# archinetai/audio-diffusion-pytorch

Hardware: AMD Instinct MI355X
Metric: denoising steps/s (UNetV0 fwd+bwd) at [B,2,2**18] (higher is better)
Workload: dtype f32; 1 GPU; BASELINE.json configs[1]: unconditional DiffusionModel(UNetV0 channels=[8,32,64,128,256,512,512,1024,1024], factors=[1,4,4,4,2,2,2,2,2], items=[1,2,2,2,2,2,2,4,4]) fwd+bwd, audio=randn(4,2,2**18) per GPU, random-init weights; per_gpu_batch=4, global_batch=4, length=262144, launch=hipGraph replay, parallelism=single, collective_world_size=1, collectives_in_graph=False, optimizer=none (the metric is fwd+bwd; gradients for all 176M parameters are produced)

## Files before the change

audio_diffusion_pytorch_amd/_C.py:

```python
import ctypes
import os
from ctypes import POINTER, Structure, c_float, c_int, c_int64, c_void_p

import torch

_PKG_DIR = os.path.dirname(os.path.abspath(__file__))
LIB_PATH = os.path.join(_PKG_DIR, "libadp_hip.so")

_lib = None
_allow_cpu = False

ERRORS = {-1: "bad shape", -2: "unsupported configuration", -3: "misaligned pointer", -4: "kernel launch failed",
          -5: "null pointer"}

P = c_void_p
I = c_int64
F = c_float


class ConvDesc(Structure):
    _fields_ = [(n, c_void_p) for n in ("x", "x2", "w", "bias", "pro_stats", "pro_gamma", "pro_beta", "e_scale",
                                        "res", "out", "out_pre")] + \
               [(n, c_int64) for n in ("B", "R", "R1", "Lin", "M", "N", "KT", "stride", "dil", "pad", "up",
                                       "transposed", "prologue", "groups", "store", "sp", "e_bstride")] + \
# ... 79 lines not shown
    "adp_tflat_out_len": (I, [I, I, I]),
    "adp_tflat_fwd": (c_int, [P, P, I, I, I, I, I, P, P]),
    "adp_tflat_wgrad_ws_bytes": (I, [I, I, I, I, I]),
    "adp_tflat_wgrad": (c_int, [P, P, I, I, I, I, I, P, P, P]),
    "adp_ctx_fold_fwd": (c_int, [P, P, P, I, I, I, P, P, P]),
    "adp_ctx_fold_bwd": (c_int, [P, P, P, P, P, I, I, I, P, P, P, P]),
    "adp_attn_fwd": (c_int, [P, P, P, I, I, I, I, I, I, I, P, P, P, P]),
    "adp_attn_fwd_ws_bytes": (I, [I, I, I, I, I]),
    "adp_attn_bwd_ws_bytes": (I, [I, I, I, I, I]),
    "adp_attn_bwd": (c_int, [P, P, P, P, P, P, I, I, I, I, I, I, I, P, P, P, P, P]),
    "adp_probe_copy": (c_int, [P, P, I, P]),
    "adp_probe_mfma": (I, [I, P, I, P]),
    "adp_probe_launch": (c_int, [I, P]),
    "adp_probe_chase": (c_int, [P, I, P, P]),
    "adp_probe_copy_v": (c_int, [P, P, I, c_int, P]),
    "adp_probe_mfma_v": (I, [I, P, I, c_int, P]),
}

ABI["adp_ar.h"] = {
    "adp_arv_noise": (c_int, [P, P, P, I, I, I, I, P, P, P, P]),
    "adp_arv_step": (c_int, [P, P, P, I, I, I, I, P, P, P]),
    "adp_arv_plane": (c_int, [P, I, I, I, P, P]),
}

ABI["adp_lt.h"] = {
    "adp_lt_conv_out_len": (I, [I, I, I, I]),
    "adp_lt_convt_out_len": (I, [I, I, I, I]),
    "adp_lt_conv": (c_int, [P, P, I, I, I, I, I, I, I, I, P, P]),
    "adp_lt_convt": (c_int, [P, P, I, I, I, I, I, I, I, I, I, P, P]),
    "adp_lt_wgrad_ws_bytes": (I, [I, I, I, I, I]),
    "adp_lt_wgrad": (c_int, [P, P, I, I, I, I, I, I, I, I, I, P, P, P]),
}

ABI["adp_enc.h"] = {
    "adp_enc_down_out_len": (I, [I, I]),
    "adp_enc_down_fwd": (c_int, [P, P, P, I, I, I, I, I, P, P]),
    "adp_enc_down_dgrad": (c_int, [P, P, I, I, I, I, I, P, P]),
    "adp_enc_down_wgrad_ws_bytes": (I, [I, I, I, I, I]),
    "adp_enc_down_wgrad": (c_int, [P, P, I, I, I, I, I, P, P, P, P]),
    "adp_enc_tanh_fwd": (c_int, [P, I, P, P]),
    "adp_enc_tanh_bwd": (c_int, [P, P, I, P, P]),
}

ABI["adp_t5.h"] = {
    "adp_t5_embed": (c_int, [P, P, I, I, I, P, P]),
    "adp_t5_rmsnorm": (c_int, [P, P, I, I, F, P, P]),
    "adp_t5_linear_ws_bytes": (I, [I, I, I]),
    "adp_t5_linear": (c_int, [P, P, P, I, I, I, I, P, P, P]),
    "adp_t5_attn": (c_int, [P, P, P, P, I, I, I, I, I, P, P]),
}

ABI["adp_rng.h"] = {
    "adp_philox_bits": (c_int, [P, I, P, P]),
    "adp_randn": (c_int, [P, I, P, P]),
    "adp_v_inpaint_step_rng": (c_int, [P, P, P, P, P, P, I, P, P]),
}

ABI["adp_clip.h"] = {
    "adp_clip_ws_bytes": (I, [I, I]),
    "adp_clip_scale": (c_int, [P, P, P, I, I, I, F, F, P, P, P]),
    "adp_clip_apply": (c_int, [P, P, I, I, P, P]),
    "adp_clip_step": (c_int, [P, P, P, P, P, I, P, I, I, P, P, P, P]),
}

ABI["adp_gated.h"] = {
    "adp_gated_linear_ws_bytes": (I, [I, I, I]),
    "adp_gated_linear": (c_int, [P, P, P, I, I, I, I, P, P, P]),
}

ABI["adp_sde.h"] = {
    "adp_v_step_eta": (c_int, [P, P, P, P, I, P, I, I, P, P]),
}

ABI["adp_rf.h"] = {
    "adp_rf_noise": (c_int, [P, P, P, I, I, P, P, P]),
    "adp_rf_step": (c_int, [P, P, P, P, I, I, P, I, I, P, P, P]),
}

ABI["adp_edm.h"] = {
    "adp_edm_noise": (c_int, [P, P, P, F, I, I, P, P, P]),
    "adp_edm_step": (c_int, [P, P, P, P, P, I, I, P, I, I, P, P, P]),
}


HEADER_SOURCE = {"adp_ar.h": "elementwise.hip", "adp_lt.h": "lt.hip", "adp_enc.h": "encoder.hip", "adp_t5.h": "t5.hip",
                 "adp_rng.h": "rng.hip", "adp_clip.h": "clip.hip", "adp_gated.h": "gated.hip", "adp_sde.h": "sde.hip",
                 "adp_rf.h": "rf.hip", "adp_edm.h": "edm.hip"}

SIGNATURES = {}
for _header, _table in ABI.items():
    for _name in _table:
        if _name in SIGNATURES:
            _first = next(h for h, t in ABI.items() if _name in t)
            raise ImportError(f"{_name} is in the tables of both {_first} and {_header}: one header declares an entry point")
    SIGNATURES.update(_table)


def _bind(path: str):
    lib = ctypes.CDLL(path)
    for name, (res, args) in SIGNATURES.items():
        fn = getattr(lib, name)
        fn.restype = res
        fn.argtypes = args
    return lib


def lib():
    global _lib
    if _lib is None:
        if not os.path.exists(LIB_PATH):
            raise RuntimeError(
                f"{LIB_PATH} is missing: build the gfx950 kernels first "
                "(python -m audio_diffusion_pytorch_amd.build or __graft_entry__.build()); "
                "audio_diffusion_pytorch_amd has no CPU/PyTorch fallback path")
        _lib = _bind(LIB_PATH)
    return _lib


def _testing_use_library(path, allow_cpu: bool):
    global _lib, _allow_cpu
    _lib = _bind(path) if path is not None else None
    _allow_cpu = allow_cpu


def stream() -> int:
    if _allow_cpu and not torch.cuda.is_available():
        return 0
    return torch.cuda.current_stream().cuda_stream


def ptr(t, dtype=torch.float32):
    if t is None:
        return None
    if t.dtype != dtype:
        raise TypeError(f"adp kernel argument must be {dtype}; got {t.dtype}")
    if not t.is_contiguous():
        raise ValueError("adp kernels need contiguous tensors")
    if not t.is_cuda and not _allow_cpu:
        raise RuntimeError("adp kernels run on MI355X (HIP) tensors only; got a CPU tensor and there is no CPU path")
    return t.data_ptr()


def check(code: int, what: str):
    if code != 0:
        raise RuntimeError(f"{what} failed: {ERRORS.get(code, code)} ({code})")


PROFILE = None
_TAG = None
REPLAY = None


def tag(**meta):
    global _TAG
    if PROFILE is not None:
        _TAG = meta


def _decode_trace(text: str) -> str:
    import re
    names = []
    for item in text.split("\n"):
        if not item:
            continue
        kern, _, site = item.partition("@")
        kern = kern.strip()
        while kern.startswith("(") and kern.endswith(")"):
            kern = kern[1:-1].strip()
        m = re.search(r"\[(?:with )?([^\]]*)\]\s*$", site)
        env = {}
# ... 60 lines not shown
```

audio_diffusion_pytorch_amd/build.py:

```python
import glob
import os
import subprocess
import sys

PKG_DIR = os.path.dirname(os.path.abspath(__file__))
REPO_ROOT = os.path.dirname(PKG_DIR)
CSRC = os.path.join(PKG_DIR, "csrc")
LIB_PATH = os.path.join(PKG_DIR, "libadp_hip.so")
SOURCES = ["conv1d.hip", "conv_mm.hip", "conv_mm_m64.hip", "conv_mm_m32.hip", "conv_tile.hip", "conv_tilek.hip", "conv_tilek1.hip", "conv_mm4.hip", "wgrad_mm.hip", "conv_direct.hip", "wgrad_direct.hip", "norm.hip", "elementwise.hip", "resample.hip", "linear.hip", "attention.hip", "ctx_bank.hip", "lt.hip", "encoder.hip", "t5.hip", "gated.hip", "rng.hip", "clip.hip", "sde.hip", "rf.hip", "edm.hip", "probe.hip"]


def _newest_mtime(paths):
    return max(os.path.getmtime(p) for p in paths)


def sources():
    return [os.path.join(CSRC, s) for s in SOURCES if os.path.exists(os.path.join(CSRC, s))]


def headers():
    return sorted(glob.glob(os.path.join(CSRC, "*.h")) + glob.glob(os.path.join(REPO_ROOT, "include", "*.h")))


def build(force: bool = False, verbose: bool = True) -> str:
    srcs = sources()
    deps = srcs + headers()
    if not force and os.path.exists(LIB_PATH) and os.path.getmtime(LIB_PATH) >= _newest_mtime(deps):
        return LIB_PATH
    hipcc = os.environ.get("HIPCC", "/opt/rocm/bin/hipcc")
    objs = []
    procs = []
    os.makedirs(os.path.join(PKG_DIR, "build"), exist_ok=True)
    for s in srcs:
        o = os.path.join(PKG_DIR, "build", os.path.basename(s) + ".o")
        objs.append(o)
        if not force and os.path.exists(o) and os.path.getmtime(o) >= _newest_mtime([s] + deps[len(srcs):]):
            continue
        cmd = [hipcc, "--offload-arch=gfx950", "-O3", "-std=c++17", "-fPIC", "-c", "-x", "hip", s, "-o", o,
               "-I", os.path.join(REPO_ROOT, "include"), "-I", CSRC, "-Wno-unused-value"]
        if verbose:
            print("[adp build]", " ".join(cmd), flush=True)
        procs.append((cmd, subprocess.Popen(cmd)))
    for cmd, p in procs:
        if p.wait() != 0:
            raise RuntimeError("hipcc failed: " + " ".join(cmd))
    cmd = [hipcc, "--offload-arch=gfx950", "-shared", "-fPIC", "-o", LIB_PATH] + objs
    if verbose:
        print("[adp build]", " ".join(cmd), flush=True)
    subprocess.check_call(cmd)
    return LIB_PATH


if __name__ == "__main__":
    build(force="--force" in sys.argv)
```

audio_diffusion_pytorch_amd/ops.py:

```python
import contextlib
import ctypes
import os
from ctypes import byref
from typing import Optional, Tuple

import torch
from torch import Tensor

from . import _C
from ._C import ConvDesc, WgradDesc, ptr

GN_EPS = 1e-5
MODULATION_LN_EPS = 1e-5
ATTENTION_LN_EPS = 1e-5


def _ws(nbytes: int, like: Tensor) -> Tensor:
    return torch.empty(max(1, (nbytes + 3) // 4), dtype=torch.float32, device=like.device)


def conv_out_len(Lin: int, KT: int, stride: int, dil: int, pad: int, up: int) -> int:
    return (Lin * up + 2 * pad - dil * (KT - 1) - 1) // stride + 1


def conv1d(x: Tensor, w: Tensor, bias: Optional[Tensor] = None, *, stride: int = 1, dil: int = 1, pad: int = 0,
           up: int = 1, transposed: bool = False, x2: Optional[Tensor] = None, prologue: int = 0,
           pro_stats: Optional[Tensor] = None, pro_gamma: Optional[Tensor] = None, pro_beta: Optional[Tensor] = None,
           groups: int = 1, e_scale: Optional[Tensor] = None, e_bstride: int = 0, res: Optional[Tensor] = None,
           store: int = 0, sp: int = 1, N: Optional[int] = None, out: Optional[Tensor] = None,
           out_pre: Optional[Tensor] = None, gn: Optional["GnPart"] = None, gnb: Optional["GnBwdPart"] = None) -> Tensor:
    B, R1, Lin = x.shape
    R = R1 + (x2.shape[1] if x2 is not None else 0)
    if transposed:
        Rw, M, KT = w.shape
    else:
        M, Rw, KT = w.shape
    assert Rw == R, f"weight expects {Rw} input channels, got {R}"
    if N is None:
        N = conv_out_len(Lin, KT, stride, dil, pad, up)
    if store == 0:
        oshape = (B, M, N)
    elif store == 1:
        oshape = (B, M // sp, N * sp)
    else:
        oshape = (B, M, N // sp)
    if out is None:
        out = torch.empty(oshape, dtype=torch.float32, device=x.device)
    else:
        assert tuple(out.shape) == oshape, (out.shape, oshape)
    d = ConvDesc(ptr(x), ptr(x2), ptr(w), ptr(bias), ptr(pro_stats), ptr(pro_gamma), ptr(pro_beta), ptr(e_scale),
                 ptr(res), ptr(out), ptr(out_pre), B, R, R1, Lin, M, N, KT, stride, dil, pad, up, int(transposed), prologue, groups,
                 store, sp, e_bstride, None, None)
    need = _C.query("adp_conv1d_ws_bytes", byref(d))
    if need > 0:
        ws = _ws(need, x)
        d.ws = ptr(ws)
    if gn is not None:
        E = _C.query("adp_conv1d_gn_entries", byref(d))
        if E > 0:
            gn.part = torch.empty((B, M // 4, E, 3), dtype=torch.float32, device=x.device)
            gn.of = out
            d.gn_part = ptr(gn.part)
    if gnb is not None and GNB_EPILOGUE:
        d.gnb_groups = gnb.groups
        d.gnb_x, d.gnb_stats, d.gnb_gamma, d.gnb_beta = ptr(gnb.x), ptr(gnb.stats), ptr(gnb.gamma), ptr(gnb.beta)
        E = _C.query("adp_conv1d_gnb_entries", byref(d))
        if E > 0:
            gnb.ab = torch.empty((B, M, E, 2), dtype=torch.float32, device=x.device)
            d.gnb_ab = ptr(gnb.ab)
    if _C.PROFILE is not None:
        _C.tag(flops=2 * B * M * N * R * KT,
               bytes=4 * (B * R * Lin + out.numel() + w.numel() + (res.numel() if res is not None else 0)),
               shape=f"B{B} R{R} M{M} N{N} KT{KT} s{stride} up{up} tr{int(transposed)} pro{prologue}")
    _C.call("adp_conv1d", byref(d), _C.stream())
    if _C.REPLAY is not None:
        keep = (x, x2, w, bias, pro_stats, pro_gamma, pro_beta, e_scale, res, out, out_pre, gn.part if gn is not None else None,
                (gnb.x, gnb.stats, gnb.gamma, gnb.beta, gnb.ab) if gnb is not None else None, ws if need > 0 else None)
        _C.REPLAY.append((f"B{B} R{R} M{M} N{N} KT{KT} s{stride} up{up} tr{int(transposed)} pro{prologue}",
                          4 * (B * R * Lin + out.numel() + w.numel() + (res.numel() if res is not None else 0)),
                          lambda d=d, keep=keep: _C.call("adp_conv1d", byref(d), _C.stream())))
    return out


class WgradPark:

    BATCH_BYTES = 80 << 20

    SIDE = os.environ.get("ADP_WGRAD_SIDE", "0") != "0"
    _side_streams = {}

    def __init__(self):
        self.items = []
        self.calls = []
        self.held = []
        self.forked = None
        if "ADP_WGRAD_BATCH_MB" in os.environ:
            self.BATCH_BYTES = int(os.environ["ADP_WGRAD_BATCH_MB"]) << 20

    def _fork(self, t: Tensor):
        if not (self.SIDE and t.is_cuda):
            return contextlib.nullcontext()
        side = self.forked
        if side is None:
            side = self._side_streams.get(t.device)
            if side is None:
                side = self._side_streams[t.device] = torch.cuda.Stream(device=t.device)
            self.forked = side
        side.wait_stream(torch.cuda.current_stream(t.device))
        return torch.cuda.stream(side)

    def join(self) -> None:
        if self.forked is not None:
            torch.cuda.current_stream(self.forked.device).wait_stream(self.forked)
            self.forked = None
            self.held.clear()

    def add(self, key, ws: Tensor, dw: Tensor, dbias: Optional[Tensor]) -> None:
        self.items.append((key, ws, dw, dbias))

    def add_call(self, key, d: WgradDesc, keep) -> None:
        self.calls.append((key, d, keep))

    def flush(self) -> None:
        if not self.calls and not self.items:
            return
        with self._fork(self.calls[0][2][0] if self.calls else self.items[0][1]):
            self._flush()

    def _flush(self) -> None:
        if self.calls:
            groups = {}
            for key, d, keep in self.calls:
                groups.setdefault(key, []).append(d)
            calls, self.calls = self.calls, []
            for key, ds in groups.items():
                arr = (WgradDesc * len(ds))(*ds)
                if _C.PROFILE is not None:
                    B, R, _, Lin, M, N, KT = key[:7]
                    _C.tag(flops=2 * B * M * N * R * KT * len(ds), bytes=4 * len(ds) * (B * R * Lin + B * M * N + M * R * KT),
                           shape=f"n{len(ds)} B{B} R{R} M{M} N{N} KT{KT}")
                _C.call("adp_conv1d_wgrad_batch", arr, len(ds), _C.stream())
            if self.forked is not None:
                self.held.append(calls)
            del calls
        if not self.items:
            return
        groups = {}
        for key, ws, dw, dbias in self.items:
            groups.setdefault(key, []).append((ws, dw, dbias))
        if self.forked is not None:
            self.held.append(self.items)
        self.items = []
        for (partials, cnt, M, acc, has_bias), g in groups.items():
            n = len(g)
            arr = ctypes.c_void_p * n
            wsa, dwa = arr(*[ptr(t[0]) for t in g]), arr(*[ptr(t[1]) for t in g])
            dba = arr(*[ptr(t[2]) for t in g]) if has_bias else None
            _C.tag(bytes=4 * n * (partials + 1) * (cnt + M), shape=f"n{n} P{partials} cnt{cnt}")
            _C.call("adp_wgrad_reduce_batch", wsa, dwa, dba, n, partials, cnt, M, acc, _C.stream())


def conv1d_wgrad(x: Tensor, dy: Tensor, KT: int, *, stride: int = 1, dil: int = 1, pad: int = 0, up: int = 1,
                 x2: Optional[Tensor] = None, prologue: int = 0, pro_stats: Optional[Tensor] = None,
# ... 1181 lines not shown
```

audio_diffusion_pytorch_amd/unet.py:

```python
from typing import Dict, List, Optional, Sequence

import os

import torch
import torch.nn as nn
from torch import Tensor

from . import ops
from .attention import PendingLN

ITEM_RESNET = "resnet"
ITEM_MODULATION = "modulation"
ITEM_INJECT = "inject"
ITEM_ATTENTION = "attention"
ITEM_CROSS_ATTENTION = "cross_attention"

TIME_EMBED_DIM = 256
TIME_NUM_LAYERS = 2
ACT_NONE, ACT_SILU, ACT_GELU = 0, 1, 2

A_UNET_SEMANTICS = {
    "DOWNSAMPLE_WIDTH": 1,
    "UPSAMPLE_KERNEL_SIZE": 3,
    "RESNET_KERNEL_SIZE": 3,
# ... 306 lines not shown

    def ctx_final_depth(self) -> int:
        for d, its in enumerate(self.item_types):
            if ITEM_CROSS_ATTENTION in its:
                return d
        return -1

    def block_param_range(self, d: int):
        cache = self.__dict__.setdefault("_block_ranges", {})
        if d not in cache:
            t = self._param_offsets()
            spans = [v for k, v in t.items() if k.startswith(f"blocks.{d}.") and not self._is_ctx_side(k)]
            cache[d] = (min(a for a, _ in spans), max(b for _, b in spans))
        return cache[d]

    def nonblock_param_ranges(self):
        if getattr(self, "_nonblock_ranges", None) is None:
            t = self._param_offsets()
            spans = sorted(v for k, v in t.items() if not k.startswith("blocks.") and k != "bank_weight")
            out = []
            for a, b in spans:
                if out and out[-1][1] == a:
                    out[-1] = (out[-1][0], b)
                else:
                    out.append((a, b))
            self._nonblock_ranges = out
        return self._nonblock_ranges

    def forward(self, x: Tensor, time: Optional[Tensor] = None, *, features: Optional[Tensor] = None,
                embedding: Optional[Tensor] = None, channels: Optional[Sequence[Optional[Tensor]]] = None,
                x_append: Optional[Tensor] = None, conditioning: Optional[Tensor] = None) -> Tensor:
        if conditioning is not None:
            if torch.is_grad_enabled() and (x.requires_grad or any(p.requires_grad for _, p in self._named_params())):
                raise RuntimeError("UNetV0.forward(conditioning=...) is an inference-only path (torch.no_grad())")
            assert features is None and conditioning.shape == (x.shape[0], self.bank_total), \
                "conditioning: [B, bank_total] rows of conditioning_table, without `features`"
        if self.use_time:
            assert time is not None, "TimeConditioningPlugin requires time in forward"
        elif time is not None:
            raise TypeError("UNetV0(use_time_conditioning=False).forward() takes 1 positional argument (x); "
                            "`time` was given")
        if self.bank_total > 0 and not self.use_time:
            assert features is not None, "ModulationItem requires `features` when use_time_conditioning=False"
        params = [p for _, p in self._named_params()]
        ctx_list = [c for c in (channels or []) if c is not None]
        grad_on = torch.is_grad_enabled()
        if not x.is_cuda:
            return _UNetFn.apply(self, x, time, features, embedding, x_append, channels, len(ctx_list), conditioning,
                                 grad_on, *ctx_list, *params)
        for t in (time, features, embedding, x_append, conditioning, *ctx_list, params[0]):
            if t is not None and t.device != x.device:
                raise RuntimeError(f"UNetV0: every tensor must live on the input's device {x.device}; got {t.device}")
        with torch.cuda.device(x.device):
            return _UNetFn.apply(self, x, time, features, embedding, x_append, channels, len(ctx_list), conditioning,
                                 grad_on, *ctx_list, *params)

    @torch.no_grad()
    def conditioning_table(self, times: Tensor) -> Optional[Tensor]:
        if not (self.use_time and self.bank_total > 0):
            return None
        run = _Run(self, False)
        return run.conditioning(times.reshape(-1), None)


NATIVE_FACTORS = (1, 2, 4)
SKIP_CAT_SCALE = 2 ** -0.5
POISON_GRADS = os.environ.get("ADP_DEBUG_POISON", "0") == "1"
GN_EPILOGUE = int(os.environ.get("ADP_GN_EPILOGUE", "1"))


def _grad_buffer(shape, device) -> Tensor:
    buf = torch.empty(shape, dtype=torch.float32, device=device)
    if POISON_GRADS:
        buf.fill_(float("nan"))
    return buf


MOD_LN_FUSE = os.environ.get("ADP_MOD_LN_FUSE", "1") != "0"

MOD_LN_BWD_FUSE = os.environ.get("ADP_MOD_LN_BWD_FUSE", "1") != "0"

ACT_MATERIALIZE_MIN_C = int(os.environ.get("ADP_ACT_MATERIALIZE_MIN_C", "64"))


class _Run:

    def __init__(self, net: UNetV0Net, need_grad: bool):
        self.net = net
        self.need_grad = need_grad
        self.tape: List = []
        self.grads: Dict[str, Tensor] = {}
        net._named_params()
        self.pnames = net._pname_cache
        self.gn: Optional[ops.GnPart] = None
        self.ln_ready = None
        self.mod_sums = ops.ModulationSums()
        self.wpark = ops.WgradPark() if os.environ.get("ADP_WGRAD_PARK", "1") != "0" else None

    def g(self, p: nn.Parameter) -> Tensor:
        try:
            return self.grads[self.pnames[id(p)]]
        except KeyError:
            raise RuntimeError("UNetV0: a parameter the kernels read is not one of the net's registered Parameters (replaced "
                               "between forward and backward, or wrapped by nn.utils.parametrize -- not supported by the "
                               "one-node U-Net: its gradient would have no slot in the flat gradient buffer)") from None

    def gspan(self, p_first: nn.Parameter, numel: int) -> Tensor:
        a, _ = self.net._param_offsets()[self.pnames[id(p_first)]]
        return self.flat[a:a + numel]

    def conditioning(self, time: Tensor, features: Optional[Tensor], ss_pre: Optional[Tensor] = None):
        n = self.net
        self.ss_all = self.dss_all = None
        if ss_pre is not None:
            assert not self.need_grad
            self.feats = None
            self.ss_all = ss_pre.contiguous()
            return self.ss_all
        if n.use_time:
            t = time.reshape(-1).to(torch.float32).contiguous()
            four = ops.time_fourier_fwd(t, n.time_weights)
            pre = [ops.linear_fwd(four, n.time_linear.weight, n.time_linear.bias)]
            acts = [ops.act_fwd(pre[0], ACT_GELU)]
            for lin in n.time_mlp:
                pre.append(ops.linear_fwd(acts[-1], lin.weight, lin.bias))
                acts.append(ops.act_fwd(pre[-1], ACT_GELU))
            feats = acts[-1] if features is None else ops.add(features.contiguous(), acts[-1])
            self.t, self.four, self.pre, self.acts = t, four, pre, acts
        else:
            feats = features.contiguous() if features is not None else None
        self.feats = feats
        if n.bank_total > 0:
            self.ss_all = ops.linear_fwd(feats, n.bank_weight, n.bank_bias, act=ACT_SILU)
            if self.need_grad:
                self.dss_all = _grad_buffer(self.ss_all.shape, self.ss_all.device)
        return self.ss_all

    def conditioning_backward(self) -> Tensor:
        n = self.net
        if n.bank_total == 0:
            return None
        assert not self.mod_sums.items, "dss_all is read while second stages of Modulation backwards are still parked"
        dfa = ops.linear_bwd_data(self.dss_all, n.bank_weight)
        dfeat = ops.act_bwd(self.feats, dfa, ACT_SILU)
        if not n.use_time:
            return dfeat
        dcur = dfeat
        lins = [n.time_linear] + list(n.time_mlp)
        for i in range(len(lins) - 1, -1, -1):
            dp = ops.act_bwd(self.pre[i], dcur, ACT_GELU)
            xin = self.four if i == 0 else self.acts[i - 1]
            ops.linear_bwd_weight(dp, xin, act=ACT_NONE, dw=self.g(lins[i].weight), dbias=self.g(lins[i].bias))
            dcur = ops.linear_bwd_data(dp, lins[i].weight)
        ops.time_fourier_bwd(self.t, n.time_weights, dcur, dw=self.g(n.time_weights))
        return dfeat

    def bank_grad_all(self) -> None:
        n = self.net
        if n.bank_total > 0:
            assert not self.mod_sums.items, "parked Modulation sums while the bank's gradient is formed"
            ops.linear_bwd_weight(self.dss_all.view(-1), self.feats, act=ACT_SILU, dw=self.g(n.bank_weight),
                                  dbias=self.g(n.bank_bias), rows=n.bank_total, dy_bstride=n.bank_total)

    def bank_grad_for_depth(self, d: int, defer: bool = False):
        n = self.net
        a, b = n.bank_depth_rows[d] if n.bank_total > 0 else (0, 0)
        self.mod_sums.flush(a, b)
        assert not any(a <= it[0] < b for it in self.mod_sums.items), "parked Modulation sums inside the rows being read"
        if b > a and not defer:
            K = n.mf
            ops.linear_bwd_weight(self.dss_all.view(-1)[a:], self.feats, act=ACT_SILU,
                                  dw=self.g(n.bank_weight)[a:b], dbias=self.g(n.bank_bias)[a:b], rows=b - a,
                                  dy_bstride=n.bank_total)
        return a, b

    def ss(self, key):
        off, nout = self.net.bank_slices[key]
        return self.ss_all.view(-1)[off:], (self.dss_all.view(-1)[off:] if self.need_grad else None)

    def gn_part_for(self, C: int) -> Optional[ops.GnPart]:
        if GN_EPILOGUE and (C // self.net.groups) % 4 == 0:
            return ops.GnPart()
        return None

    def gn_stats_of(self, x: Tensor) -> Tensor:
        G = self.net.groups
        if self.gn is not None and self.gn.covers(x):
            return ops.gn_finalize(self.gn.part, G)
        return ops.gn_stats(x, G)

    def gn_stats_act_of(self, x: Tensor, gnp):
        G = self.net.groups
        if self.gn is not None and self.gn.covers(x):
            part = self.gn.part
            if (x.shape[1] // G // 4) * part.shape[2] <= 1024:
                return ops.gn_finalize_act(x, part, G, gnp.weight, gnp.bias)
            st = ops.gn_finalize(part, G)
            return st, ops.gn_act(x, st, G, gnp.weight, gnp.bias)
        return ops.gn_stats_act(x, G, gnp.weight, gnp.bias)

    def resnet(self, p, x: Tensor) -> Tensor:
        G = self.net.groups
        if x.shape[1] >= ACT_MATERIALIZE_MIN_C and x.shape[0] * x.shape[1] <= 65535:
            return self.resnet_wide(p, x)
        st1 = self.gn_stats_of(x)
        self.gn = self.gn_part_for(x.shape[1])
        h1 = ops.conv1d(x, p.conv1.weight, p.conv1.bias, pad=1, prologue=1, pro_stats=st1, pro_gamma=p.gn1.weight,
                        pro_beta=p.gn1.bias, groups=G, gn=self.gn)
        st2 = self.gn_stats_of(h1)
        self.gn = None
        y = ops.conv1d(h1, p.conv2.weight, p.conv2.bias, pad=1, prologue=1, pro_stats=st2, pro_gamma=p.gn2.weight,
                       pro_beta=p.gn2.bias, groups=G, res=x)
        if self.need_grad:
            def bwd(gy):
                ops.conv1d_wgrad(h1, gy, 3, pad=1, park=self.wpark, prologue=1, pro_stats=st2, pro_gamma=p.gn2.weight,
                                 pro_beta=p.gn2.bias, groups=G, dw=self.g(p.conv2.weight), dbias=self.g(p.conv2.bias))
                gb2 = ops.GnBwdPart(h1, st2, p.gn2.weight, p.gn2.bias, G)
                dact2 = ops.conv1d(gy, p.conv2.weight, None, pad=1, transposed=True, gnb=gb2)
                dh1, _, _ = ops.gn_silu_bwd(h1, dact2, st2, p.gn2.weight, p.gn2.bias, G, dgamma=self.g(p.gn2.weight),
                                            dbeta=self.g(p.gn2.bias), ab=gb2.ab)
                ops.conv1d_wgrad(x, dh1, 3, pad=1, park=self.wpark, prologue=1, pro_stats=st1, pro_gamma=p.gn1.weight,
                                 pro_beta=p.gn1.bias, groups=G, dw=self.g(p.conv1.weight), dbias=self.g(p.conv1.bias))
                gb1 = ops.GnBwdPart(x, st1, p.gn1.weight, p.gn1.bias, G)
                dact1 = ops.conv1d(dh1, p.conv1.weight, None, pad=1, transposed=True, gnb=gb1)
                dx, _, _ = ops.gn_silu_bwd(x, dact1, st1, p.gn1.weight, p.gn1.bias, G, dres=gy,
                                           dgamma=self.g(p.gn1.weight), dbeta=self.g(p.gn1.bias), ab=gb1.ab)
                return dx
            self.tape.append((bwd, None))
        return y

    def resnet_wide(self, p, x: Tensor) -> Tensor:
        G = self.net.groups
        st1, a1 = self.gn_stats_act_of(x, p.gn1)
        self.gn = self.gn_part_for(x.shape[1])
        h1 = ops.conv1d(a1, p.conv1.weight, p.conv1.bias, pad=1, gn=self.gn)
        st2, a2 = self.gn_stats_act_of(h1, p.gn2)
        self.gn = None
        y = ops.conv1d(a2, p.conv2.weight, p.conv2.bias, pad=1, res=x)
        if self.need_grad:
            def bwd(gy):
                ops.conv1d_wgrad(a2, gy, 3, pad=1, dw=self.g(p.conv2.weight), dbias=self.g(p.conv2.bias), park=self.wpark)
                gb2 = ops.GnBwdPart(h1, st2, p.gn2.weight, p.gn2.bias, G)
                dact2 = ops.conv1d(gy, p.conv2.weight, None, pad=1, transposed=True, gnb=gb2)
                dh1, _, _ = ops.gn_silu_bwd(h1, dact2, st2, p.gn2.weight, p.gn2.bias, G, dgamma=self.g(p.gn2.weight),
                                            dbeta=self.g(p.gn2.bias), ab=gb2.ab)
                ops.conv1d_wgrad(a1, dh1, 3, pad=1, dw=self.g(p.conv1.weight), dbias=self.g(p.conv1.bias), park=self.wpark)
                gb1 = ops.GnBwdPart(x, st1, p.gn1.weight, p.gn1.bias, G)
                dact1 = ops.conv1d(dh1, p.conv1.weight, None, pad=1, transposed=True, gnb=gb1)
                dx, _, _ = ops.gn_silu_bwd(x, dact1, st1, p.gn1.weight, p.gn1.bias, G, dres=gy,
                                           dgamma=self.g(p.gn1.weight), dbeta=self.g(p.gn1.bias), ab=gb1.ab)
                return dx
            self.tape.append((bwd, None))
        return y

    def modulation(self, key, x: Tensor, attn_next=None) -> Tensor:
        ss, dss = self.ss(key)
        NT = self.net.bank_total
        self.gn = None
        if attn_next is not None and MOD_LN_FUSE:
            p, dual = attn_next
            y, stats, xn, cn, st = ops.modulation_ln_fwd(x, ss, NT, p.norm.weight, p.norm.bias,
                                                         p.norm_context.weight if dual else None,
                                                         p.norm_context.bias if dual else None)
            self.ln_ready = (y, xn, cn, st)
        else:
            y, stats = ops.modulation_fwd(x, ss, NT)
        if self.need_grad:
            off = self.net.bank_slices[key][0]

            def bwd(gy):
                if isinstance(gy, PendingLN):
                    return self.mod_sums.partial_ln(off, x, ss, NT, stats, dss, NT, gy.y, gy.dxn, gy.gamma, gy.ln_stats,
                                                    gy.dres, gy.dgb)
                return self.mod_sums.partial(off, x, gy, ss, NT, stats, dss, NT)
            self.tape.append((bwd, None))
        return y

    def inject(self, p, x: Tensor, ctx: Tensor, ctx_index: int) -> Tensor:
        assert ctx.shape[0] == x.shape[0] and ctx.shape[2] == x.shape[2], "context `channels` shape mismatch"
        ctx = ctx.contiguous()
        y = ops.conv1d(x, p.conv.weight, p.conv.bias, x2=ctx, res=x)
        if self.need_grad:
            def bwd(gy):
                ops.conv1d_wgrad(x, gy, 1, x2=ctx, dw=self.g(p.conv.weight), dbias=self.g(p.conv.bias))
                C = x.shape[1]
                w = p.conv.weight
                dx = ops.conv1d(gy, w[:, :C, :].contiguous(), None, transposed=True, res=gy)
                if self.ctx_grads is not None and self.ctx_needs[ctx_index]:
                    prev = self.ctx_grads[ctx_index]
                    self.ctx_grads[ctx_index] = ops.conv1d(gy, w[:, C:, :].contiguous(), None, transposed=True, res=prev)
                return dx
            self.tape.append((bwd, None))
        return y

    def attention(self, p, x: Tensor, context: Optional[Tensor]) -> Tensor:
        from . import attention as attn_host
        return attn_host.attention_item(self, p, x, context)

    def run_items(self, d: int, which: str, mods, x: Tensor, embedding, channels) -> Tensor:
        if self.need_grad and self.wpark is not None:
            self.tape.append((self._flush_wpark, None))
        for i, (t, p) in enumerate(zip(self.net.item_types[d], mods)):
            if t == ITEM_RESNET:
                x = self.resnet(p, x)
            elif t == ITEM_MODULATION:
                nxt = self.net.item_types[d][i + 1] if i + 1 < len(mods) else None
                attn_next = (mods[i + 1], nxt == ITEM_ATTENTION) if nxt in (ITEM_ATTENTION, ITEM_CROSS_ATTENTION) else None
                x = self.modulation((d, which, i), x, attn_next)
            elif t == ITEM_INJECT:
                assert channels is not None and channels[d] is not None, f"Missing context `channels` at depth {d}"
                x = self.inject(p, x, channels[d], self.ctx_index[d])
            elif t == ITEM_ATTENTION:
                x = self.attention(p, x, None)
            elif t == ITEM_CROSS_ATTENTION:
                assert embedding is not None, "You must provide a context when using context_features"
                x = self.attention(p, x, embedding)
        return x

    def _flush_wpark(self, gy):
        self.wpark.flush()
        return gy

    def block(self, d: int, x: Tensor, x2: Optional[Tensor], embedding, channels, need_dx: bool) -> Tensor:
        n = self.net
        if d == len(n.blocks):
            return x
        blk = n.blocks[d]
        f, NT = n.factors[d], n.bank_total
        native = f in NATIVE_FACTORS
        has_adapter = hasattr(blk, "skip_adapter")
        if has_adapter:
# ... 197 lines not shown
```

Measured before the change: 92.40 denoising steps/s.

## Add Winograd F(4,3) MFMA conv kernel for 64-channel resnet convolutions

Introduces a Winograd-transformed 3-tap conv kernel for 64-channel stride-1 convolutions. Weights are transformed in LDS and the six transformed points are multiplied with MFMA. Bias, residual, GroupNorm partial statistics and GN-backward partial sums are fused into the epilogue. Wide resnet blocks route their forward and transposed backward convs through it when the activation is large enough. This cuts multiply work, at the cost of Winograd's float rounding differences and a new specialized code path.

```diff
diff --git a/audio_diffusion_pytorch_amd/_C.py b/audio_diffusion_pytorch_amd/_C.py
--- a/audio_diffusion_pytorch_amd/_C.py
+++ b/audio_diffusion_pytorch_amd/_C.py
@@ -185,10 +185,17 @@
     "adp_edm_step": (c_int, [P, P, P, P, P, I, I, P, I, I, P, P, P]),
 }
 
+ABI["adp_tilec.h"] = {
+    "adp_tilec_eligible": (I, [POINTER(ConvDesc)]),
+    "adp_tilec_gn_entries": (I, [POINTER(ConvDesc)]),
+    "adp_tilec_gnb_entries": (I, [POINTER(ConvDesc)]),
+    "adp_tilec_conv": (c_int, [POINTER(ConvDesc), P]),
+}
+
 
 HEADER_SOURCE = {"adp_ar.h": "elementwise.hip", "adp_lt.h": "lt.hip", "adp_enc.h": "encoder.hip", "adp_t5.h": "t5.hip",
                  "adp_rng.h": "rng.hip", "adp_clip.h": "clip.hip", "adp_gated.h": "gated.hip", "adp_sde.h": "sde.hip",
-                 "adp_rf.h": "rf.hip", "adp_edm.h": "edm.hip"}
+                 "adp_rf.h": "rf.hip", "adp_edm.h": "edm.hip", "adp_tilec.h": "conv_tilec.hip"}
 
 SIGNATURES = {}
 for _header, _table in ABI.items():
diff --git a/audio_diffusion_pytorch_amd/build.py b/audio_diffusion_pytorch_amd/build.py
--- a/audio_diffusion_pytorch_amd/build.py
+++ b/audio_diffusion_pytorch_amd/build.py
@@ -7,7 +7,7 @@
 REPO_ROOT = os.path.dirname(PKG_DIR)
 CSRC = os.path.join(PKG_DIR, "csrc")
 LIB_PATH = os.path.join(PKG_DIR, "libadp_hip.so")
-SOURCES = ["conv1d.hip", "conv_mm.hip", "conv_mm_m64.hip", "conv_mm_m32.hip", "conv_tile.hip", "conv_tilek.hip", "conv_tilek1.hip", "conv_mm4.hip", "wgrad_mm.hip", "conv_direct.hip", "wgrad_direct.hip", "norm.hip", "elementwise.hip", "resample.hip", "linear.hip", "attention.hip", "ctx_bank.hip", "lt.hip", "encoder.hip", "t5.hip", "gated.hip", "rng.hip", "clip.hip", "sde.hip", "rf.hip", "edm.hip", "probe.hip"]
+SOURCES = ["conv1d.hip", "conv_mm.hip", "conv_mm_m64.hip", "conv_mm_m32.hip", "conv_tile.hip", "conv_tilec.hip", "conv_tilek.hip", "conv_tilek1.hip", "conv_mm4.hip", "wgrad_mm.hip", "conv_direct.hip", "wgrad_direct.hip", "norm.hip", "elementwise.hip", "resample.hip", "linear.hip", "attention.hip", "ctx_bank.hip", "lt.hip", "encoder.hip", "t5.hip", "gated.hip", "rng.hip", "clip.hip", "sde.hip", "rf.hip", "edm.hip", "probe.hip"]
 
 
 def _newest_mtime(paths):
diff --git a/audio_diffusion_pytorch_amd/csrc/conv_tilec.hip b/audio_diffusion_pytorch_amd/csrc/conv_tilec.hip
--- /dev/null
+++ b/audio_diffusion_pytorch_amd/csrc/conv_tilec.hip
@@ -0,0 +1,331 @@
+#include <stdlib.h>
+#include "adp_rt.h"
+#include "adp.h"
+#include "adp_tilec.h"
+
+namespace {
+
+constexpr int TC_KT = 3;
+constexpr int TC_TN = 64;
+constexpr int TC_RS = TC_TN + 2;
+constexpr int TC_XC = 32;
+constexpr int TC_XT = TC_XC * TC_RS;
+constexpr int TC_MR = 32;
+
+template <int C, bool TR, int NW, bool RES, bool GN, bool GNB>
+__global__ __launch_bounds__(64 * NW) void conv_tilec_kernel(adp_conv_desc d, int tiles_per_b) {
+  constexpr int NH = C / TC_MR;
+  constexpr int NCH = C / TC_XC;
+  constexpr int US = C * 2 * 16 * 6;
+  __shared__ __attribute__((aligned(16))) float lds[US + NW * 16 + NW * TC_XT];
+  float* const us = lds;
+  float* const gsh = lds + US;
+  float* const xs = gsh + NW * 16;
+  const int tid = threadIdx.x, lane = tid & 63;
+  const int wave = adp_uniform(tid >> 6);
+  const int j = lane & 15, kq = lane >> 4;
+  const int L = (int)d.Lin;
+  const int g = (int)blockIdx.x / NH, rh = (int)blockIdx.x - g * NH;
+  const int co = TC_MR * rh;
+  const int t = g * NW + wave;
+  const int b = t / tiles_per_b;
+  const int n0 = (t - b * tiles_per_b) * TC_TN;
+  const int64_t xbase = (int64_t)b * C * L + n0;
+  const int64_t obase = xbase + (int64_t)co * L;
+  const unsigned Lb = 4u * (unsigned)L;
+
+  const char* xt = reinterpret_cast<const char*>(d.x + xbase);
+  f32x4 rx[8];
+  const int hi = lane >> 5, l31 = lane & 31;
+  const int hrel = hi ? TC_TN : -1;
+  const bool hok = n0 + hrel >= 0 && n0 + hrel < L;
+  float hx = 0.0f;
+  const unsigned ldb = (unsigned)(lane >> 4) * Lb + 16u * (unsigned)(lane & 15);
+  const unsigned hb = (unsigned)l31 * Lb + 4u * (unsigned)(hok ? hrel + 1 : 1);
+  auto load_chunk = [&](int h) {
+    const unsigned cb = (unsigned)(TC_XC * h) * Lb;
+#pragma unroll
+    for (int i = 0; i < 8; ++i) rx[i] = *reinterpret_cast<const f32x4*>(xt + (cb + ldb + 4u * (unsigned)i * Lb));
+    hx = *reinterpret_cast<const float*>(xt - 4 + (cb + hb));
+  };
+
+  {
+    constexpr int NT = 64 * NW, NIT = TC_MR * C / NT, HB = NIT < 8 ? NIT : 8;
+    static_assert(NIT * NT == TC_MR * C && NIT % HB == 0, "the workgroup's threads divide the weight pairs");
+#pragma unroll 1
+    for (int k0 = 0; k0 < NIT; k0 += HB) {
+      float wv[HB][3];
+#pragma unroll
+      for (int k = 0; k < HB; ++k) {
+        const int p = tid + (k0 + k) * NT, q = p >> 4;
+        const int c = q % C, ml = (p & 15) + 16 * (q / C);
+        const float* wp = d.w + (TR ? (int64_t)c * C + co + ml : (int64_t)(co + ml) * C + c) * TC_KT;
+#pragma unroll
+        for (int q3 = 0; q3 < 3; ++q3) wv[k][q3] = wp[q3];
+      }
+      if (k0 == 0) load_chunk(0);
+#pragma unroll
+      for (int k = 0; k < HB; ++k) {
+        const int p = tid + (k0 + k) * NT, q = p >> 4;
+        const int c = q % C, ml = (p & 15) + 16 * (q / C);
+        const float a = wv[k][0], g1 = wv[k][1], e = wv[k][2];
+        const float g0 = TR ? e : a, g2 = TR ? a : e;
+        const float s02 = g0 + g2, qq = 0.041666666666666664f * g0 + 0.16666666666666666f * g2;
+        float* u = us + ((c * 2 + (ml >> 4)) * 16 + (ml & 15)) * 6;
+        *reinterpret_cast<f32x2*>(u) = f32x2{0.25f * g0, -0.16666666666666666f * (s02 + g1)};
+        *reinterpret_cast<f32x2*>(u + 2) = f32x2{-0.16666666666666666f * (s02 - g1), qq + 0.08333333333333333f * g1};
+        *reinterpret_cast<f32x2*>(u + 4) = f32x2{qq - 0.08333333333333333f * g1, g2};
+      }
+    }
+  }
+  adp_barrier_lds();
+
+  f32x4 M[2][6];
+#pragma unroll
+  for (int rb = 0; rb < 2; ++rb)
+#pragma unroll
+    for (int p = 0; p < 6; ++p) M[rb][p] = f32x4{0.0f, 0.0f, 0.0f, 0.0f};
+  float* X = xs + wave * TC_XT;
+  const float* Xr = X + kq * TC_RS + 4 * j;
+  const float* Ur = us + (kq * 32 + j) * 6;
+#pragma unroll
+  for (int h = 0; h < NCH; ++h) {
+    if (h > 0) adp_wave_sync();
+    {
+      float* o = X + (lane >> 4) * TC_RS + 4 * (lane & 15) + 1;
+#pragma unroll
+      for (int i = 0; i < 8; ++i) {
+        o[4 * i * TC_RS] = rx[i][0];
+        *reinterpret_cast<f32x2*>(o + 4 * i * TC_RS + 1) = f32x2{rx[i][1], rx[i][2]};
+        o[4 * i * TC_RS + 3] = rx[i][3];
+      }
+      X[l31 * TC_RS + (hi ? TC_RS - 1 : 0)] = hok ? hx : 0.0f;
+    }
+    adp_wave_sync();
+    if (h + 1 < NCH) load_chunk(h + 1);
+    const float* Uh = Ur + h * TC_XC * 192;
+    f32x2 dn[3], un[2][3];
+    auto frags = [&](int ks) {
+#pragma unroll
+      for (int q = 0; q < 3; ++q) {
+        dn[q] = *reinterpret_cast<const f32x2*>(Xr + 4 * ks * TC_RS + 2 * q);
+        un[0][q] = *reinterpret_cast<const f32x2*>(Uh + 4 * ks * 192 + 2 * q);
+        un[1][q] = *reinterpret_cast<const f32x2*>(Uh + 4 * ks * 192 + 96 + 2 * q);
+      }
+    };
+    frags(0);
+#pragma unroll
+    for (int ks = 0; ks < TC_XC / 4; ++ks) {
+      f32x2 dc[3], uc[2][3];
+#pragma unroll
+      for (int q = 0; q < 3; ++q) {
+        dc[q] = dn[q];
+        uc[0][q] = un[0][q];
+        uc[1][q] = un[1][q];
+      }
+      if (ks + 1 < TC_XC / 4) frags(ks + 1);
+      adp_sched_fence();
+      const float d0 = dc[0][0], d1 = dc[0][1], d2 = dc[1][0], d3 = dc[1][1], d4 = dc[2][0], d5 = dc[2][1];
+      const float a = fmaf(-4.0f, d2, d4), bb = fmaf(-4.0f, d1, d3), c = d4 - d2, e = 2.0f * (d3 - d1);
+      float v[6];
+      v[0] = fmaf(4.0f, d0, fmaf(-5.0f, d2, d4));
+      v[1] = a + bb;
+      v[2] = a - bb;
+      v[3] = c + e;
+      v[4] = c - e;
+      v[5] = fmaf(4.0f, d1, fmaf(-5.0f, d3, d5));
+#pragma unroll
+      for (int p = 0; p < 6; ++p) {
+        M[0][p] = adp_mfma16(uc[0][p >> 1][p & 1], v[p], M[0][p]);
+        M[1][p] = adp_mfma16(uc[1][p >> 1][p & 1], v[p], M[1][p]);
+      }
+      adp_sched_fence();
+    }
+  }
+
+  char* ot = reinterpret_cast<char*>(d.out + obase);
+  const char* rt = reinterpret_cast<const char*>(RES ? d.res + obase : d.out + obase);
+  const unsigned ob = 4u * (unsigned)kq * Lb + 16u * (unsigned)j;
+  const int E = tiles_per_b / NW, ei = g - b * E;
+#pragma unroll
+  for (int rb = 0; rb < 2; ++rb) {
+    f32x4 rv[4], bv = f32x4{0.0f, 0.0f, 0.0f, 0.0f};
+    if (RES) {
+#pragma unroll
+      for (int r = 0; r < 4; ++r) rv[r] = *reinterpret_cast<const f32x4*>(rt + (ob + (unsigned)(16 * rb + r) * Lb));
+    }
+    if (d.bias) bv = *reinterpret_cast<const f32x4*>(d.bias + co + 16 * rb + 4 * kq);
+    f32x4 gxq[4], gga = bv, gbe = bv;
+    if (GNB) {
+      const char* gxt = reinterpret_cast<const char*>(d.gnb_x + obase);
+#pragma unroll
+      for (int r = 0; r < 4; ++r) gxq[r] = *reinterpret_cast<const f32x4*>(gxt + (ob + (unsigned)(16 * rb + r) * Lb));
+      gga = *reinterpret_cast<const f32x4*>(d.gnb_gamma + co + 16 * rb + 4 * kq);
+      gbe = *reinterpret_cast<const f32x4*>(d.gnb_beta + co + 16 * rb + 4 * kq);
+    }
+    float gk = 0.0f;
+    f32x2 gs = f32x2{0.0f, 0.0f}, gq = f32x2{0.0f, 0.0f};
+#pragma unroll
+    for (int r = 0; r < 4; ++r) {
+      const float m0 = M[rb][0][r], m1 = M[rb][1][r], m2 = M[rb][2][r], m3 = M[rb][3][r], m4 = M[rb][4][r], m5 = M[rb][5][r];
+      const float s12 = m1 + m2, d12 = m1 - m2, s34 = m3 + m4, d34 = m3 - m4;
+      f32x2 ya = f32x2{m0 + s12 + s34, fmaf(2.0f, d34, d12)} + bv[r];
+      f32x2 yb = f32x2{fmaf(4.0f, s34, s12), fmaf(8.0f, d34, d12) + m5} + bv[r];
+      if (RES) {
+        ya = ya + f32x2{rv[r][0], rv[r][1]};
+        yb = yb + f32x2{rv[r][2], rv[r][3]};
+      }
+      *reinterpret_cast<f32x4*>(ot + (ob + (unsigned)(16 * rb + r) * Lb)) = f32x4{ya[0], ya[1], yb[0], yb[1]};
+      if (GNB) {
+        const int cl = 16 * rb + 4 * kq + r;
+        const float* st = d.gnb_stats + ((int64_t)b * d.gnb_groups + (co + cl) / (C / (int)d.gnb_groups)) * 2;
+        const float mu = st[0], rs = st[1];
+        const float ga = gga[r] * rs, be = gbe[r] - mu * ga;
+        const float yv[4] = {ya[0], ya[1], yb[0], yb[1]};
+        float sa = 0.0f, sb = 0.0f;
+#pragma unroll
+        for (int k = 0; k < 4; ++k) {
+          const float xh = (gxq[r][k] - mu) * rs;
+          const float ds = yv[k] * adp_dsilu_fast(fmaf(gxq[r][k], ga, be));
+          sa = fmaf(ds, xh, sa);
+          sb += ds;
+        }
+        sa = adp_row16_sum(sa), sb = adp_row16_sum(sb);
+        if (j == 0) *reinterpret_cast<f32x2*>(X + 2 * cl) = f32x2{sa, sb};
+      }
+      if (GN) {
+        if (r == 0) gk = __shfl(ya[0], lane & 48, 64);
+        const f32x2 ea = ya - gk, eb = yb - gk;
+        gs = gs + ea + eb;
+        gq = ea * ea + (eb * eb + gq);
+      }
+    }
+    if (GN) {
+      constexpr float cnt = 4.0f * TC_TN;
+      const float sv = adp_row16_sum(gs[0] + gs[1]), qv = adp_row16_sum(gq[0] + gq[1]);
+      if (j == 0) {
+        float* e = gsh + (wave * 8 + 4 * rb + kq) * 2;
+        e[0] = gk + sv / cnt;
+        e[1] = fmaxf(qv - sv * (sv / cnt), 0.0f);
+      }
+    }
+  }
+  if (GNB) {
+    __syncthreads();
+    if (tid < TC_MR) {
+      float sa = 0.0f, sb = 0.0f;
+      for (int w = 0; w < NW; ++w) {
+        const f32x2 p = *reinterpret_cast<const f32x2*>(xs + w * TC_XT + 2 * tid);
+        sa += p[0], sb += p[1];
+      }
+      *reinterpret_cast<f32x2*>(d.gnb_ab + (((int64_t)b * C + co + tid) * E + ei) * 2) = f32x2{sa, sb};
+    }
+  }
+  if (GN) {
+    constexpr float cnt = 4.0f * TC_TN;
+    __syncthreads();
+    if (tid < 8) {
+      float mean = gsh[tid * 2], m2 = gsh[tid * 2 + 1], n = cnt;
+      for (int w = 1; w < NW; ++w) {
+        const float mw = gsh[(w * 8 + tid) * 2], dl = mw - mean, nn = n + cnt;
+        mean += dl * (cnt / nn);
+        m2 += gsh[(w * 8 + tid) * 2 + 1] + dl * dl * (n * cnt / nn);
+        n = nn;
+      }
+      float* e = d.gn_part + (((int64_t)b * (C / 4) + 8 * rh + tid) * E + ei) * 3;
+      e[0] = mean;
+      e[1] = m2;
+      e[2] = n;
+    }
+  }
+}
+
+bool off16(const void* p) { return (reinterpret_cast<uintptr_t>(p) & 15) != 0; }
+bool off4(const void* p) { return (reinterpret_cast<uintptr_t>(p) & 3) != 0; }
+
+bool tilec_channels(int64_t c) { return c == 64; }
+
+bool tilec_shape(const adp_conv_desc& d) {
+  if (!tilec_channels(d.R) || d.R1 != d.R || d.M != d.R || d.KT != TC_KT) return false;
+  if (d.stride != 1 || d.dil != 1 || d.pad != 1 || d.up != 1 || d.store != 0 || d.prologue != 0) return false;
+  if (d.out_pre || d.e_scale || d.x2) return false;
+  if (d.B < 1 || d.Lin < TC_TN || d.N != d.Lin || d.N % TC_TN != 0) return false;
+  if (d.B * (d.N / TC_TN) >= (int64_t)1 << 28 || d.B * d.R * d.Lin >= (int64_t)1 << 40) return false;
+  if ((d.R + 1) * d.Lin * 4 >= (int64_t)1 << 32) return false;
+  if (d.transposed && (d.res || d.gn_part)) return false;
+  return true;
+}
+
+bool tilec_gnb_shape(const adp_conv_desc& d) {
+  return d.transposed && !d.bias && d.gnb_x && d.gnb_stats && d.gnb_gamma && d.gnb_beta && d.gnb_groups >= 1 &&
+         d.R % d.gnb_groups == 0;
+}
+
+int tilec_check(const adp_conv_desc& d) {
+  if (!d.x || !d.w || !d.out) return ADP_ERR_NULL;
+  if (d.B < 0 || d.R < 0 || d.M < 0 || d.Lin < 0 || d.N < 0) return ADP_ERR_SHAPE;
+  if (!tilec_shape(d)) return ADP_ERR_UNSUPPORTED;
+  if (d.gnb_ab && !tilec_gnb_shape(d)) return ADP_ERR_UNSUPPORTED;
+  if (off16(d.x) || off16(d.out) || off16(d.res) || off16(d.bias) || off4(d.w) || off4(d.gn_part)) return ADP_ERR_ALIGN;
+  if (d.gnb_ab && (off16(d.gnb_x) || off16(d.gnb_gamma) || off16(d.gnb_beta) || off4(d.gnb_stats) ||
+                   (reinterpret_cast<uintptr_t>(d.gnb_ab) & 7)))
+    return ADP_ERR_ALIGN;
+  return ADP_OK;
+}
+
+int tilec_nw(const adp_conv_desc& d) {
+  const int64_t tiles_per_b = d.N / TC_TN, groups = tiles_per_b * d.B * (d.R / TC_MR);
+  const char* e = adp_knob_raw("ADP_TILEC_NW");
+  const int want = e ? atoi(e) : 8;
+  for (int nw : {8, 2})
+    if (nw <= want && tiles_per_b % nw == 0 && (e || groups / nw >= 256)) return nw;
+  return 1;
+}
+
+template <int C, bool TR, bool RES, bool GN, bool GNB>
+int launch_tilec(const adp_conv_desc& d, void* stream) {
+  const int tiles_per_b = (int)(d.N / TC_TN);
+  const int nw = tilec_nw(d);
+  const unsigned grid = (unsigned)(d.B * tiles_per_b / nw * (C / TC_MR));
+  switch (nw) {
+    case 8: ADP_LAUNCH((conv_tilec_kernel<C, TR, 8, RES, GN, GNB>), dim3(grid), dim3(512), stream, d, tiles_per_b); break;
+    case 2: ADP_LAUNCH((conv_tilec_kernel<C, TR, 2, RES, GN, GNB>), dim3(grid), dim3(128), stream, d, tiles_per_b); break;
+    default: ADP_LAUNCH((conv_tilec_kernel<C, TR, 1, RES, GN, GNB>), dim3(grid), dim3(64), stream, d, tiles_per_b); break;
+  }
+  return ADP_LAUNCH_OK();
+}
+
+template <int C>
+int launch_tilec_c(const adp_conv_desc& d, void* stream) {
+  if (d.gnb_ab) return launch_tilec<C, true, false, false, true>(d, stream);
+  if (d.transposed) return launch_tilec<C, true, false, false, false>(d, stream);
+  if (d.res) return d.gn_part ? launch_tilec<C, false, true, true, false>(d, stream) : launch_tilec<C, false, true, false, false>(d, stream);
+  return d.gn_part ? launch_tilec<C, false, false, true, false>(d, stream) : launch_tilec<C, false, false, false, false>(d, stream);
+}
+
+}
+
+extern "C" int64_t adp_tilec_eligible(const adp_conv_desc* d) {
+  if (!d) return ADP_ERR_NULL;
+  return tilec_check(*d) == ADP_OK ? 1 : 0;
+}
+
+extern "C" int64_t adp_tilec_gn_entries(const adp_conv_desc* d) {
+  if (!d) return ADP_ERR_NULL;
+  if (tilec_check(*d) != ADP_OK || d->transposed) return 0;
+  return d->N / TC_TN / tilec_nw(*d);
+}
+
+extern "C" int64_t adp_tilec_gnb_entries(const adp_conv_desc* d) {
+  if (!d) return ADP_ERR_NULL;
+  if (tilec_check(*d) != ADP_OK || !tilec_gnb_shape(*d)) return 0;
+  if (off16(d->gnb_x) || off16(d->gnb_gamma) || off16(d->gnb_beta) || off4(d->gnb_stats)) return 0;
+  return d->N / TC_TN / tilec_nw(*d);
+}
+
+extern "C" int adp_tilec_conv(const adp_conv_desc* d, void* stream) {
+  if (!d) return ADP_ERR_NULL;
+  const int code = tilec_check(*d);
+  if (code != ADP_OK) return code;
+  return launch_tilec_c<64>(*d, stream);
+}
diff --git a/audio_diffusion_pytorch_amd/ops.py b/audio_diffusion_pytorch_amd/ops.py
--- a/audio_diffusion_pytorch_amd/ops.py
+++ b/audio_diffusion_pytorch_amd/ops.py
@@ -79,6 +79,54 @@
         _C.REPLAY.append((f"B{B} R{R} M{M} N{N} KT{KT} s{stride} up{up} tr{int(transposed)} pro{prologue}",
                           4 * (B * R * Lin + out.numel() + w.numel() + (res.numel() if res is not None else 0)),
                           lambda d=d, keep=keep: _C.call("adp_conv1d", byref(d), _C.stream())))
+    return out
+
+
+def conv_tilec(x: Tensor, w: Tensor, bias: Optional[Tensor] = None, *, stride: int = 1, pad: int = 1,
+               transposed: bool = False, res: Optional[Tensor] = None, out: Optional[Tensor] = None, gn: Optional["GnPart"] = None,
+               gnb: Optional["GnBwdPart"] = None) -> Optional[Tensor]:
+    B, R, Lin = x.shape
+    if transposed:
+        Rw, M, KT = w.shape
+    else:
+        M, Rw, KT = w.shape
+    assert Rw == R, f"weight expects {Rw} input channels, got {R}"
+    N = conv_out_len(Lin, KT, stride, 1, pad, 1)
+    if N < 1 or (transposed and (res is not None or gn is not None)):
+        return None
+    if out is None:
+        out = torch.empty((B, M, N), dtype=torch.float32, device=x.device)
+    else:
+        assert tuple(out.shape) == (B, M, N), (out.shape, (B, M, N))
+    d = ConvDesc(ptr(x), None, ptr(w), ptr(bias), None, None, None, None, ptr(res), ptr(out), None, B, R, R, Lin, M, N, KT,
+                 stride, 1, pad, 1, int(transposed), 0, 1, 0, 1, 0, None, None)
+    if _C.query("adp_tilec_eligible", byref(d)) == 0:
+        return None
+    part = ab = None
+    if gn is not None:
+        E = _C.query("adp_tilec_gn_entries", byref(d))
+        if E > 0:
+            part = torch.empty((B, M // 4, E, 3), dtype=torch.float32, device=x.device)
+            d.gn_part = ptr(part)
+    if gnb is not None and GNB_EPILOGUE:
+        d.gnb_groups = gnb.groups
+        d.gnb_x, d.gnb_stats, d.gnb_gamma, d.gnb_beta = ptr(gnb.x), ptr(gnb.stats), ptr(gnb.gamma), ptr(gnb.beta)
+        E = _C.query("adp_tilec_gnb_entries", byref(d))
+        if E > 0:
+            ab = torch.empty((B, M, E, 2), dtype=torch.float32, device=x.device)
+            d.gnb_ab = ptr(ab)
+    label = f"B{B} R{R} M{M} N{N} KT{KT} s{stride} up1 tr{int(transposed)} pro0"
+    nbytes = 4 * (B * R * Lin + out.numel() + w.numel() + (res.numel() if res is not None else 0))
+    if _C.PROFILE is not None:
+        _C.tag(flops=2 * B * M * N * R * KT, bytes=nbytes, shape=label)
+    _C.call("adp_tilec_conv", byref(d), _C.stream())
+    if gn is not None and part is not None:
+        gn.part, gn.of = part, out
+    if gnb is not None:
+        gnb.ab = ab
+    if _C.REPLAY is not None:
+        keep = (x, w, bias, res, out, part, (gnb.x, gnb.stats, gnb.gamma, gnb.beta, ab) if gnb is not None else None)
+        _C.REPLAY.append((label, nbytes, lambda d=d, keep=keep: _C.call("adp_tilec_conv", byref(d), _C.stream())))
     return out
 
 
diff --git a/audio_diffusion_pytorch_amd/unet.py b/audio_diffusion_pytorch_amd/unet.py
--- a/audio_diffusion_pytorch_amd/unet.py
+++ b/audio_diffusion_pytorch_amd/unet.py
@@ -412,6 +412,21 @@
 
 ACT_MATERIALIZE_MIN_C = int(os.environ.get("ADP_ACT_MATERIALIZE_MIN_C", "64"))
 
+def tilec_on() -> bool:
+    return os.environ.get("ADP_TILEC", "1") != "0"
+
+
+def tilec_min_elems() -> int:
+    return int(os.environ.get("ADP_TILEC_MIN_ELEMS", str(1 << 22)))
+
+
+def conv_block_conv(x: Tensor, w: Tensor, bias: Optional[Tensor], **kw) -> Tensor:
+    if tilec_on() and x.numel() >= tilec_min_elems():
+        y = ops.conv_tilec(x, w, bias, pad=1, **kw)
+        if y is not None:
+            return y
+    return ops.conv1d(x, w, bias, pad=1, **kw)
+
 
 class _Run:
 
@@ -563,20 +578,20 @@
         G = self.net.groups
         st1, a1 = self.gn_stats_act_of(x, p.gn1)
         self.gn = self.gn_part_for(x.shape[1])
-        h1 = ops.conv1d(a1, p.conv1.weight, p.conv1.bias, pad=1, gn=self.gn)
+        h1 = conv_block_conv(a1, p.conv1.weight, p.conv1.bias, gn=self.gn)
         st2, a2 = self.gn_stats_act_of(h1, p.gn2)
         self.gn = None
-        y = ops.conv1d(a2, p.conv2.weight, p.conv2.bias, pad=1, res=x)
+        y = conv_block_conv(a2, p.conv2.weight, p.conv2.bias, res=x)
         if self.need_grad:
             def bwd(gy):
                 ops.conv1d_wgrad(a2, gy, 3, pad=1, dw=self.g(p.conv2.weight), dbias=self.g(p.conv2.bias), park=self.wpark)
                 gb2 = ops.GnBwdPart(h1, st2, p.gn2.weight, p.gn2.bias, G)
-                dact2 = ops.conv1d(gy, p.conv2.weight, None, pad=1, transposed=True, gnb=gb2)
+                dact2 = conv_block_conv(gy, p.conv2.weight, None, transposed=True, gnb=gb2)
                 dh1, _, _ = ops.gn_silu_bwd(h1, dact2, st2, p.gn2.weight, p.gn2.bias, G, dgamma=self.g(p.gn2.weight),
                                             dbeta=self.g(p.gn2.bias), ab=gb2.ab)
                 ops.conv1d_wgrad(a1, dh1, 3, pad=1, dw=self.g(p.conv1.weight), dbias=self.g(p.conv1.bias), park=self.wpark)
                 gb1 = ops.GnBwdPart(x, st1, p.gn1.weight, p.gn1.bias, G)
-                dact1 = ops.conv1d(dh1, p.conv1.weight, None, pad=1, transposed=True, gnb=gb1)
+                dact1 = conv_block_conv(dh1, p.conv1.weight, None, transposed=True, gnb=gb1)
                 dx, _, _ = ops.gn_silu_bwd(x, dact1, st1, p.gn1.weight, p.gn1.bias, G, dres=gy,
                                            dgamma=self.g(p.gn1.weight), dbeta=self.g(p.gn1.bias), ab=gb1.ab)
                 return dx
diff --git a/include/adp_tilec.h b/include/adp_tilec.h
--- /dev/null
+++ b/include/adp_tilec.h
@@ -0,0 +1,20 @@
+#ifndef ADP_TILEC_H
+#define ADP_TILEC_H
+#include "adp.h"
+
+#ifdef __cplusplus
+extern "C" {
+#endif
+
+int64_t adp_tilec_eligible(const adp_conv_desc* d);
+
+int64_t adp_tilec_gn_entries(const adp_conv_desc* d);
+
+int64_t adp_tilec_gnb_entries(const adp_conv_desc* d);
+
+int adp_tilec_conv(const adp_conv_desc* d, void* stream);
+
+#ifdef __cplusplus
+}
+#endif
+#endif
```

Result: no change. 93.05 denoising steps/s, median of 6 (+0.7%).
